# JonasGeiping/breaching

Measured on AMD Instinct MI355X. Metric: attack iters/sec, ResNet-18 ImageNet invertinggradients; PSNR vs ref, higher is better.
Workload: dtype f32

## Files before the change

breaching_amd/_lib.py:

```python

import ctypes
import os
from ctypes import POINTER, Structure, c_char_p, c_double, c_float, c_int, c_int32, c_int64, c_uint32, c_void_p

from . import build as _build

BH_ABI_VERSION = 8
BH_GM_CHUNK = 4096
BH_GM_MAX_PTRS = 448
BH_GM_PARTIAL_STRIDE = 4
BH_GM_MAX_ROWS = 2048
BH_GM_DEFAULT_ROWS = 512
BH_GM_STAT_WORDS = 12
BH_PRIOR_MAX_GRID = 1024
BH_BN_MAX_LAYERS = 448
BH_MT_MAX_PTRS = 112
BH_BN_TILE = 4096
BH_PRIOR_PARTIAL_STRIDE = 2
BH_STATE_WORDS = 16
BH_SCHED_STRIDE = 4
GM_CACHE_AUTO, GM_CACHE_KEEP, GM_CACHE_STREAM, GM_CACHE_STREAM_ALL = 0, 1, 2, 3

GM_KINDS = {
    "cosine-similarity": 0,
    "masked-cosine-similarity": 1,
    "fast-cosine-similarity": 2,
    "angular": 3,
    "euclidean": 4,
    "l1": 5,
    "tag-euclidean": 6,
    "pearlmutter-loss": 7,
}
GM_STAT_PATCH_D, GM_STAT_PATCH_R, GM_STAT_FD_STEP, GM_STAT_FD_SCALE = 8, 9, 10, 11
STATE_IT, STATE_DEAD, STATE_FIRST_BAD, STATE_IMPROVED, STATE_MIN, STATE_TOTAL, STATE_GNORM = range(7)
SIGN_NONE, SIGN_HARD, SIGN_SOFT = 0, 1, 2


class GmChunk(Structure):
    _fields_ = [("flat_off", c_int64), ("tensor_off", c_int64), ("tensor", c_int32), ("len", c_int32)]


class BnLayer(Structure):
    _fields_ = [("flat_off", c_int64), ("sums_off", c_int64), ("chan_off", c_int32), ("B", c_int32), ("C", c_int32),
                ("HW", c_int32), ("S", c_int32), ("narrow", c_int32), ("weight", c_float), ("div_unit_mul", c_uint32),
                ("div_unit_shr", c_uint32), ("div_c_mul", c_uint32), ("div_c_shr", c_uint32), ("fwd_items", c_int32)]


class BnItem(Structure):
    _fields_ = [("layer", c_int32), ("a", c_int32), ("b", c_int32), ("c", c_int32)]


class PsnrParams(Structure):
    _fields_ = [("mean", c_float * 4), ("std", c_float * 4), ("factor", c_float), ("clip", c_int32)]


class StepParams(Structure):
    _fields_ = [
        ("n", c_int64),
        ("plane", c_int64),
        ("channels", c_int32),
# ... 13 lines not shown

BH_STEP_MAX_SLOTS = 4


class StepSlot(Structure):
    _fields_ = [("params", StepParams), ("x", c_void_p), ("g", c_void_p), ("g_reg", c_void_p), ("noise", c_void_p), ("m", c_void_p),
                ("v", c_void_p), ("best", c_void_p)]


_PROTOTYPES = {
    "bh_abi_version": (c_int32, []),
    "bh_build_arch": (c_char_p, []),
    "bh_gm_num_groups": (c_int32, [c_int32]),
    "bh_gm_table_size": (c_int, [c_int32, POINTER(c_int64), POINTER(c_int64), POINTER(c_int64)]),
    "bh_gm_build_table": (c_int, [c_int32, POINTER(c_int64), POINTER(GmChunk), c_int64, POINTER(c_int64)]),
    "bh_gm_group_bounds": (c_int, [c_int32, POINTER(GmChunk), c_int64, POINTER(c_int32)]),
    "bh_gm_fwd": (
        c_int,
        [c_int32, c_int32, POINTER(c_void_p), c_void_p, c_void_p, c_int64, POINTER(c_int32), c_void_p, c_float, c_void_p,
         c_int32, c_int32, c_void_p, c_void_p, c_void_p],
    ),
    "bh_gm_fwd_rows": (c_int32, [c_int32, POINTER(c_int32), c_int32]),
    "bh_gm_finalize": (
        c_int,
        [c_int32, c_void_p, c_int64, c_float, c_float, c_float, c_float, c_void_p, c_void_p, c_void_p, c_void_p, c_void_p],
    ),
    "bh_wall_clock_khz": (c_int32, []),
    "bh_gm_bwd": (
        c_int,
        [c_int32, c_int32, POINTER(c_void_p), c_void_p, c_void_p, c_int64, POINTER(c_int32), c_void_p, c_void_p, c_void_p, c_void_p, c_int32,
         c_void_p, c_void_p, c_void_p],
    ),
    "bh_gm_pack": (c_int, [c_int32, POINTER(c_void_p), c_void_p, c_int64, POINTER(c_int32), c_void_p, c_void_p]),
    "bh_prior_tv_norm": (
        c_int,
        [c_void_p, c_int32, c_int32, c_int32, c_float, c_float, c_float, c_float, c_int32, c_float, c_float, c_void_p, c_void_p, c_void_p],
    ),
    "bh_bn_plan_size": (
        c_int,
        [c_int32, POINTER(c_int32), POINTER(c_int32), POINTER(c_int32), POINTER(c_int64), POINTER(c_int64), POINTER(c_int64),
         POINTER(c_int64), POINTER(c_int64)],
    ),
    "bh_bn_plan_build": (
        c_int,
        [c_int32, POINTER(c_int32), POINTER(c_int32), POINTER(c_int32), POINTER(c_float), POINTER(BnLayer), POINTER(BnItem),
         c_int64, POINTER(BnItem), c_int64],
    ),
    "bh_bn_bwd_accumulate": (c_int, [c_void_p, c_void_p, c_int32, c_void_p, c_void_p, c_int64, c_void_p, c_void_p, c_void_p, c_void_p]),
    "bh_bn_eval_fwd": (c_int, [c_void_p] * 8 + [c_int32, c_int32, c_int32, c_int32, c_void_p]),
    "bh_bn_eval_slabs": (c_int32, [c_int32, c_int32, c_int32]),
    "bh_bn_eval_bwd": (c_int, [c_void_p] * 14 + [c_int32, c_int32, c_int32, c_void_p]),
    "bh_bn_eval_bwd_bwd": (c_int, [c_void_p] * 14 + [c_int32, c_int32, c_int32, c_void_p]),
    "bh_bn_eval_bwd_bwd2": (c_int, [c_void_p] * 15 + [c_int32, c_int32, c_int32, c_void_p]),
    "bh_ln_fwd": (c_int, [c_void_p] * 6 + [c_int32, c_int32, ctypes.c_float, c_void_p]),
    "bh_ln_bwd": (c_int, [c_void_p] * 8 + [c_int32, c_int32, c_void_p]),
    "bh_ln_bwd_bwd": (c_int, [c_void_p] * 12 + [c_int32, c_int32, c_void_p]),
    "bh_bn_sums": (c_int, [c_int32, POINTER(c_void_p), POINTER(c_int32), c_void_p, c_void_p, c_int64, c_void_p, c_int32, c_int32, c_void_p]),
    "bh_bn_finalize": (c_int, [c_int32, c_void_p, c_void_p, c_void_p, c_void_p, c_void_p, c_void_p, c_void_p, c_void_p, c_int32, c_void_p]),
    "bh_bn_bwd": (
        c_int,
        [c_int32, POINTER(c_void_p), POINTER(c_int32), c_void_p, c_void_p, c_int64, c_void_p, c_void_p, c_void_p, c_void_p],
    ),
    "bh_mt_num_groups": (c_int32, [c_int32]),
    "bh_mt_group_bounds": (c_int, [c_int32, POINTER(GmChunk), c_int64, POINTER(c_int32)]),
    "bh_mt_axpy": (
        c_int,
        [c_int32, POINTER(c_void_p), POINTER(c_void_p), POINTER(c_void_p), c_float, c_void_p, c_int64, POINTER(c_int32), c_void_p,
         c_void_p],
    ),
    "bh_mt_scale": (c_int, [c_int32, POINTER(c_void_p), c_float, c_void_p, c_int64, POINTER(c_int32), c_void_p, c_void_p]),
    "bh_mt_patch": (
        c_int,
        [c_int32, POINTER(c_void_p), POINTER(c_void_p), c_void_p, c_void_p, c_float, c_void_p, c_int64, POINTER(c_int32), c_void_p,
         c_void_p],
    ),
    "bh_prior_orthogonality": (c_int, [c_void_p, c_int32, c_int64, c_void_p, c_void_p, c_void_p]),
    "bh_metric_psnr": (
        c_int,
        [c_void_p, c_void_p, c_int32, c_int64, c_int64, c_int32, POINTER(PsnrParams), c_void_p, c_void_p, c_void_p],
    ),
    "bh_event_create": (c_int, [POINTER(c_void_p)]),
    "bh_event_destroy": (c_int, [c_void_p]),
    "bh_event_record": (c_int, [c_void_p, c_void_p]),
    "bh_event_elapsed_ms": (c_int, [c_void_p, c_void_p, POINTER(c_float)]),
    "bh_state_reset": (c_int, [c_void_p, c_void_p]),
    "bh_loss_commit": (c_int, [c_void_p, c_void_p, c_int32, c_void_p, c_void_p, c_int32, c_void_p, c_void_p, c_void_p]),
    "bh_grad_norm": (c_int, [c_void_p, c_void_p, c_void_p, c_void_p, c_int64, c_void_p, c_float, c_void_p, c_void_p]),
    "bh_trial_key": (c_int64, [c_float, c_int32]),
    "bh_trial_key_unpack": (c_int, [c_int64, POINTER(c_float), POINTER(c_int32)]),
    "bh_step_list_norm_rows": (c_int32, [c_int32, POINTER(StepSlot)]),
    "bh_grad_norm_list": (c_int, [c_void_p, c_int32, POINTER(StepSlot), c_void_p, c_void_p, c_void_p]),
    "bh_candidate_step_list": (c_int, [c_void_p, c_void_p, c_int32, POINTER(StepSlot), c_void_p, c_void_p]),
    "bh_candidate_step": (
        c_int,
        [c_void_p, c_void_p, POINTER(StepParams), c_void_p, c_void_p, c_void_p, c_void_p, c_void_p, c_void_p, c_void_p, c_void_p],
    ),
}

EXPORTED_SYMBOLS = tuple(_PROTOTYPES)

_LIB = None


class BreachHipError(RuntimeError):
    """A C-ABI call returned a non-zero status."""

# ... 47 lines not shown
```

breaching_amd/attacker.py:

```python

import copy
import logging
import time
from collections import defaultdict

import numpy as np
import torch

from . import _lib, schedules, streams as trial_streams, trials, workers
from .config import cfg_get as _cfg_get
from .gm import objective_lookup
from .priors import HipNormRegularization, HipTotalVariation, launch_tv_norm, regularizer_lookup
from .victim_layers import (FusedEpilogueError, _ConvFunction, _ConvGradFunction, _EvalAffineBatchNorm2d, _EvalBNFunction,
                            _EvalBNGradFunction, _HipConv2d, _HipLayerNorm, owned_conv_grad_enabled, use_owned_conv_gradient,
                            _launch_eval_bn, _LayerNormFunction, _LayerNormGradFunction, _PendingBatchNorm, _under_functorch,
                            fast_eval_bn_enabled, fast_eval_bn_mode, fast_layer_norm_enabled, fuse_bn_relu_enabled, fuse_bn_relu_policy,
                            use_affine_eval_batchnorm, use_hip_layernorm)

log = logging.getLogger(__name__)

embedding_layer_names = ["encoder.weight", "word_embeddings.weight", "transformer.wte"]

_DEFAULT_SETUP = dict(dtype=torch.float, device=torch.device("cpu"))


class HipOptimizationAttacker:

    def __init__(self, model, loss_fn, cfg_attack, setup=_DEFAULT_SETUP):
        self.cfg = cfg_attack
        self.memory_format = torch.channels_last if cfg_attack.impl.mixed_precision else torch.contiguous_format
        self.setup = dict(device=torch.device(setup["device"]), dtype=getattr(torch, cfg_attack.impl.dtype))
        if self.setup["device"].type != "cuda":
            raise RuntimeError(
                f"HipOptimizationAttacker needs a ROCm device (setup['device']={self.setup['device']}); the HIP hot "
                "path has no CPU fallback. Use the reference attacker for CPU runs."
            )
        if self.setup["dtype"] != torch.float32 or cfg_attack.impl.mixed_precision:
            raise NotImplementedError("The HIP hot path computes in fp32 (impl.dtype=float, mixed_precision=False).")
        _lib.load()
        self.model_template = copy.deepcopy(model)
        self.loss_fn = copy.deepcopy(loss_fn)

        objective_cls = objective_lookup.get(self.cfg.objective.type)
        if objective_cls is None:
            raise ValueError(f"Unknown objective type {self.cfg.objective.type} given.")
        self.objective = objective_cls(**self.cfg.objective)

        self.regularizers = []
        regs = _cfg_get(self.cfg, "regularization")
        if regs is not None and hasattr(regs, "keys"):
            for key in regs.keys():
                if regs[key].scale > 0:
                    self.regularizers.append(regularizer_lookup[key](self.setup, **regs[key]))
        for reg in self.regularizers:
            if hasattr(reg, "tuning"):
                reg.tuning = {name: int(_cfg_get(self.cfg.impl, f"bn_{name}") or 0) for name in ("grid_cap", "load_depth", "finalize_block")}

        augs = _cfg_get(self.cfg, "augmentations")
        if augs is not None and hasattr(augs, "keys") and len(list(augs.keys())) > 0:
            self.augmentations = self._build_augmentations(augs, setup)
        else:
            self.augmentations = torch.nn.Sequential()

    @staticmethod
    def _build_augmentations(augs, setup):
        try:
            from breaching.attacks.auxiliaries.augmentations import augmentation_lookup
# ... 48 lines not shown
                pool.ship("starts", dict(labels=labels, inits={t: tuple(inits[t]) for t in range(num_trials) if t % pool.world != 0}),
                          self.setup["device"])
                pool.submit([dict(dryrun=dryrun)] * (pool.world - 1))
            timing["prepare_s"] = time.perf_counter() - t_call

            local_scores, local_solutions = {}, {}
            group_runs = None
            mine = list(shard.local_trials())
            width = trials_in_flight(self.cfg) if (self._fused_loop_supported() and not noisy) else 1
            try:
                for start in range(0, len(mine), max(width, 1)):
                    group = mine[start : start + max(width, 1)]
                    t_group = time.perf_counter()
                    if len(group) == 1:
                        solutions = {group[0]: self._run_trial(rec_models, shared_data, labels, stats, group[0], initial_data,
                                                               dryrun, init_state=inits.get(group[0]))}
                    else:
                        solutions, group_runs = self._run_trial_group(rec_models, shared_data, labels, stats, group, initial_data, dryrun,
                                                                      {t: inits[t] for t in group}, reuse=group_runs)
                    t_score = time.perf_counter()
                    timing["trials_s"] += t_score - t_group
                    for trial, solution in solutions.items():
                        local_solutions[trial] = solution
                        local_scores[trial] = self._score_trial(self._solution_data(solution),
                                                                self._score_labels(solution, labels), rec_models, shared_data)
                    timing["score_s"] += time.perf_counter() - t_score
            except KeyboardInterrupt:
                print("Trial procedure manually interruped.")
            if pool is not None:
                t_wait = time.perf_counter()
                pool.expect("trials_done")
                pool.timing["trials_wait_s"] = round(time.perf_counter() - t_wait, 4)
                pool.broadcast(("go",))
            before_select = getattr(self, "_before_select", None)
            if before_select is not None:
                before_select()
            stats["execution_trials"] = dict(self._trial_execution)
            t_select = time.perf_counter()
            optimal = self._select_optimal_reconstruction(local_solutions, local_scores, stats, shard)
            timing["select_s"] = time.perf_counter() - t_select
            if pool is not None:
                pool.timing["select_s"] = round(timing["select_s"], 4)
                pool.finish()
        except BaseException:
            if pool is not None:
                pool.abort()
                if pool.closed:
                    self._pool = None
            raise
        timing["total_s"] = time.perf_counter() - t_call
        stats["execution"] = dict(trials=stats.pop("execution_trials"), pool=pool.describe() if pool is not None else None,
                                  fused_epilogue_fallback=getattr(self, "fused_epilogue_fallback", None),
                                  owned_conv_grad=owned_conv_grad_enabled(self.cfg),
                                  pool_fallback=getattr(self, "_pool_fallback", None), world=shard.world,
                                  trial_streams=trial_streams.calibration_report(self.setup["device"]),
                                  timing={k: round(v, 4) for k, v in timing.items()})
        reconstructed_data = self._package(optimal, labels)
        if server_payload[0]["metadata"].modality == "text":
            raw = reconstructed_data["data"]
            reconstructed_data = self._postprocess_text_data(reconstructed_data)
            self._attach_raw_embeddings(reconstructed_data, raw)
        if "ClassAttack" in server_secrets:
            true_num_data = server_secrets["ClassAttack"]["true_num_data"]
            full = torch.zeros([true_num_data, *self.data_shape], **self.setup)
            full[server_secrets["ClassAttack"]["target_indx"]] = optimal if torch.is_tensor(optimal) else optimal[0]
            reconstructed_data["data"] = full
            reconstructed_data["labels"] = server_secrets["ClassAttack"]["all_labels"]
        return reconstructed_data, stats

    def _trial_worker_pool(self, num_trials):
        import torch.distributed as dist

        if getattr(self, "_is_trial_worker", False) or num_trials < 2:
            return None
        pool = getattr(self, "_pool", None)
        if pool is not None and not pool.closed:
            return pool
        self._pool_fallback = None
        devices = workers.requested_devices(self.cfg, self.setup["device"])[:num_trials]
        if len(devices) < 2:
            return None
        foreign = workers.active_pool()
        if foreign is not None and not foreign.busy:
            log.info("Closing another attacker's idle trial worker pool.")
            foreign.close()
        if dist.is_available() and dist.is_initialized():
            return None
        template = copy.deepcopy(self.model_template).to("cpu")
        loss_fn = copy.deepcopy(self.loss_fn).to("cpu") if isinstance(self.loss_fn, torch.nn.Module) else self.loss_fn
        try:
            self._pool = workers.TrialWorkerPool(devices, workers.attacker_runner_factory,
                                                 (type(self).__name__, template, loss_fn, self.cfg))
        except Exception as exc:
            if _cfg_get(self.cfg.impl, "trial_pool", "auto") == "required":
                raise
            self._pool_fallback = f"could not start the trial workers on devices {devices}: {exc!r}"
            log.warning(f"{self._pool_fallback}; running every trial on {self.setup['device']}.")
            self._pool = None
        return self._pool

    def close(self):
        pool = getattr(self, "_pool", None)
        if pool is not None:
            pool.close()
            self._pool = None

# ... 35 lines not shown

        metadata = server_payload[0]["metadata"]
        self.data_shape = metadata.shape
        if hasattr(metadata, "mean"):
            self.dm = torch.as_tensor(metadata.mean, **self.setup)[None, :, None, None]
            self.ds = torch.as_tensor(metadata.std, **self.setup)[None, :, None, None]
        else:
            self.dm, self.ds = torch.tensor(0, **self.setup), torch.tensor(1, **self.setup)

        rec_models = self._construct_models_from_payload_and_buffers(server_payload, shared_data)
        shared_data = self._cast_shared_data(shared_data)
        if metadata.modality == "text":
            rec_models, shared_data = self._prepare_for_text_data(shared_data, rec_models)
        self._rec_models = rec_models
        if shared_data[0]["metadata"]["labels"] is None:
            labels = self._recover_label_information(shared_data, server_payload, rec_models)
        else:
            labels = shared_data[0]["metadata"]["labels"].clone().to(self.setup["device"])
        if self.cfg.normalize_gradients:
            shared_data = self._normalize_gradients(shared_data)
        return rec_models, labels, stats

    def _construct_models_from_payload_and_buffers(self, server_payload, shared_data):
        models = []
        for idx, payload in enumerate(server_payload):
            new_model = copy.deepcopy(self.model_template)
            new_model.to(**self.setup, memory_format=self.memory_format)
            if shared_data[idx]["buffers"] is not None:
                buffers = shared_data[idx]["buffers"]
                new_model.eval()
            elif payload["buffers"] is not None:
                buffers = payload["buffers"]
                new_model.eval()
            else:
                new_model.train()
                for module in new_model.modules():
                    if hasattr(module, "track_running_stats"):
                        module.reset_parameters()
                        module.track_running_stats = False
                buffers = []
            with torch.no_grad():
                for param, server_state in zip(new_model.parameters(), payload["parameters"]):
                    param.copy_(server_state.to(**self.setup))
                for buffer, server_state in zip(new_model.buffers(), buffers):
                    buffer.copy_(server_state.to(**self.setup))
            if self.cfg.impl.JIT is not None:
                raise NotImplementedError("impl.JIT (torch.jit script/trace of the victim model) is not supported.")
            bn_mode = fast_eval_bn_mode(self.cfg)
            if bn_mode is not None:
                use_affine_eval_batchnorm(new_model, bn_mode, fuse_epilogue=fuse_bn_relu_enabled(self.cfg))
            if fast_layer_norm_enabled(self.cfg):
                use_hip_layernorm(new_model)
            if owned_conv_grad_enabled(self.cfg):
                use_owned_conv_gradient(new_model)
            models.append(new_model)
        return models

    def _cast_shared_data(self, shared_data):
        for data in shared_data:
            data["gradients"] = [g.to(**self.setup) for g in data["gradients"]]
            if data["buffers"] is not None:
                data["buffers"] = [b.to(device=self.setup["device"], dtype=self.setup["dtype"]) for b in data["buffers"]]
        return shared_data

    def _normalize_gradients(self, shared_data, fudge_factor=1e-6):
        for data in shared_data:
            grad_norm = torch.stack([g.pow(2).sum() for g in data["gradients"]]).sum().sqrt()
            torch._foreach_div_(data["gradients"], max(grad_norm, fudge_factor))
        return shared_data

    def _prepare_for_text_data(self, shared_data, rec_models):
        if self.cfg.text_strategy == "run-embedding":
            self.embeddings = []
            for model, data in zip(rec_models, shared_data):
                names = [n for n, _ in model.named_parameters()]
                name_to_idx = dict(zip(names, range(len(data["gradients"]))))
                position = None
                for marker in embedding_layer_names:
                    for key in name_to_idx:
                        if marker in key:
                            position = name_to_idx[key]
                if position is None:
                    raise ValueError("Could not locate the token embedding among the model parameters.")
                weight = list(model.parameters())[position]
                self.embeddings.append(dict(weight=weight, grads=data["gradients"].pop(position)))

                def _disable(module, weight=weight):
                    for child_name, child in module.named_children():
                        if isinstance(child, torch.nn.Embedding):
                            if child.weight is weight:
                                setattr(module, child_name, torch.nn.Identity())
                        else:
                            _disable(child)

                _disable(model)
            _, token_embedding_dim = self.embeddings[0]["weight"].shape
            self.data_shape = [*self.data_shape, token_embedding_dim]
        elif self.cfg.text_strategy == "no-preprocessing":
            pass
        else:
            raise ValueError(f"Invalid text strategy {self.cfg.text_strategy} given.")
        return rec_models, shared_data

    def _postprocess_text_data(self, reconstructed_user_data, models=None):
        def _closest_token(recovered, table):
            recovered = recovered - recovered.mean(dim=-1, keepdim=True)
            table = table - table.mean(dim=-1, keepdim=True)
# ... 801 lines not shown
```

breaching_amd/build.py:

```python

import hashlib
import os
import shutil
import subprocess
import sys

PKG_DIR = os.path.dirname(os.path.abspath(__file__))
REPO_ROOT = os.path.dirname(PKG_DIR)
CSRC = os.path.join(PKG_DIR, "csrc")
INCLUDE = os.path.join(REPO_ROOT, "include")
LIB_DIR = os.path.join(PKG_DIR, "lib")
LIB_PATH = os.path.join(LIB_DIR, "libbreach_hip.so")
STAMP_PATH = os.path.join(LIB_DIR, "libbreach_hip.stamp")

SOURCES = ["gm_kernels.hip", "prior_kernels.hip", "step_kernels.hip", "mt_kernels.hip", "affine_kernels.hip", "layernorm_kernels.hip"]
HEADERS = [os.path.join(CSRC, "bh_common.h"), os.path.join(INCLUDE, "breach_hip.h")]
ARCH = "gfx950"
FLAGS = ["-O3", "-std=c++17", "-fPIC", "-shared", f"--offload-arch={ARCH}", "-fno-gpu-rdc", "-Wall", "-Wno-unused-function"]


def _hipcc():
    for cand in (os.environ.get("HIPCC"), shutil.which("hipcc"), "/opt/rocm/bin/hipcc"):
        if cand and os.path.exists(cand):
            return cand
    raise RuntimeError("hipcc not found; libbreach_hip.so cannot be built (set HIPCC=/path/to/hipcc)")


def source_digest():
    h = hashlib.sha256()
    for path in [os.path.join(CSRC, s) for s in SOURCES] + HEADERS:
        with open(path, "rb") as f:
            h.update(f.read())
    h.update(" ".join(FLAGS).encode())
    return h.hexdigest()


def is_current():
    if not (os.path.exists(LIB_PATH) and os.path.exists(STAMP_PATH)):
        return False
    with open(STAMP_PATH) as f:
        return f.read().strip() == source_digest()


def build_library(force=False, verbose=False):
    if not force and is_current():
        return LIB_PATH
    os.makedirs(LIB_DIR, exist_ok=True)
    cmd = [_hipcc(), *FLAGS, f"-I{INCLUDE}", f"-I{CSRC}", *[os.path.join(CSRC, s) for s in SOURCES], "-o", LIB_PATH]
    if verbose:
        print(" ".join(cmd), flush=True)
    proc = subprocess.run(cmd, capture_output=True, text=True)
    if proc.returncode != 0:
        raise RuntimeError(f"hipcc failed ({proc.returncode}):\n{proc.stdout}\n{proc.stderr}")
    if verbose and proc.stderr.strip():
        print(proc.stderr, file=sys.stderr)
    with open(STAMP_PATH, "w") as f:
        f.write(source_digest())
    return LIB_PATH


if __name__ == "__main__":
    path = build_library(force="--force" in sys.argv, verbose=True)
    print(path)
```

breaching_amd/victim_layers.py:

```python

import torch

from . import _lib
from .config import cfg_get as _cfg_get

def _vector_ready(t, hw):
    if not t.is_contiguous():
        t = t.contiguous()
    if hw % 4 == 0 and t.data_ptr() % 16:
        t = t.clone()
    return t


def _under_functorch(x):
    try:
        from torch._C._functorch import is_functorch_wrapped_tensor, peek_interpreter_stack

        return bool(is_functorch_wrapped_tensor(x)) or peek_interpreter_stack() is not None
    except Exception:
        return False


class _EvalBNFunction(torch.autograd.Function):

# ... 74 lines not shown
        lib = _lib.load()
        gy, x, weight, inv_std, mean_inv, *rest = ctx.saved_tensors
        mask = rest[0] if ctx.masked else None
        none = (None,) * 9
        ggx2 = _take_conv_term(ctx)
        if ggx is None:
            ggx, ggx2 = ggx2, None
        if ggx is None and ggw is None and ggb is None and ggr is None:
            return none
        if ctx.extra_terms:
            raise NotImplementedError("No derivative of the BatchNorm backward with the DeepInversion term / another gradient folded in.")
        B, C = x.shape[0], x.shape[1]
        hw = x[0, 0].numel()
        ggx = None if ggx is None else _vector_ready(ggx.to(torch.float32), hw)
        ggx2 = None if ggx2 is None else _vector_ready(ggx2.to(torch.float32), hw)
        ggr = None if ggr is None else _vector_ready(ggr.to(torch.float32), hw)
        ggw = None if ggw is None else ggw.to(torch.float32).contiguous()
        ggb = None if ggb is None else ggb.to(torch.float32).contiguous()
        d_gy = torch.empty_like(x) if ctx.needs_input_grad[0] else None
        d_x = torch.empty_like(x) if (ctx.needs_input_grad[1] and ggw is not None) else None
        d_w = torch.empty(C, dtype=torch.float32, device=x.device) if (weight is not None and ctx.needs_input_grad[2] and ggx is not None) else None
        if d_gy is None and d_x is None and d_w is None:
            return none
        slabs = lib.bh_bn_eval_slabs(B, C, hw)
        ws = torch.empty(C * slabs, dtype=torch.float64, device=x.device) if slabs > 1 else None
        with torch.cuda.device(x.device):
            _lib.check(lib.bh_bn_eval_bwd_bwd2(_lib.ptr(ggx), _lib.ptr(ggx2), _lib.ptr(ggw), _lib.ptr(ggb), _lib.ptr(gy), _lib.ptr(x),
                                               _lib.ptr(weight), _lib.ptr(inv_std), _lib.ptr(mean_inv), _lib.ptr(d_gy), _lib.ptr(d_x),
                                               _lib.ptr(d_w), _lib.ptr(ws), _lib.ptr(mask), _lib.ptr(ggr), B, C, hw,
                                               _lib.current_stream_handle(x.device)), "bh_bn_eval_bwd_bwd2")
        return d_gy, d_x, d_w, None, None, None, None, None, None


def _take_conv_term(node):
    entry = getattr(node, "_conv_term", None)
    if entry is None:
        return None
    node._conv_term = None
    return entry[1] if entry[0] == torch._C._current_graph_task_id() else None


def _engine_wants(edge):
    node = edge[0] if edge is not None else None
    if node is None:
        return False
    try:
        return bool(torch._C._will_engine_execute_node(node))
    except RuntimeError:
        return True


_aten = torch.ops.aten


class _ConvFunction(torch.autograd.Function):

    @staticmethod
    def forward(ctx, x, w, b, stride, padding, dilation, groups):
        ctx.geometry = (list(stride), list(padding), list(dilation), int(groups))
        ctx.bias_sizes = None if b is None else [w.shape[0]]
        ctx.save_for_backward(x, w)
        return _aten.convolution(x, w, b, ctx.geometry[0], ctx.geometry[1], ctx.geometry[2], False, [0] * len(ctx.geometry[0]), groups)

    @staticmethod
    def backward(ctx, gy):
        x, w = ctx.saved_tensors
        none = (None,) * 7
        mask = tuple(bool(ctx.needs_input_grad[i]) and _engine_wants(ctx.next_functions[i]) for i in range(3))
        if not any(mask):
            return none
        producer = gy.grad_fn if gy.output_nr == 0 and getattr(gy.grad_fn, "_forward_cls", None) is _EvalBNGradFunction else None
        gx, gw, gb = _ConvGradFunction.apply(gy, x, w, ctx.geometry, mask, ctx.bias_sizes, producer)
        return (gx, gw, gb) + none[3:]


class _ConvGradFunction(torch.autograd.Function):

    @staticmethod
    def forward(ctx, gy, x, w, geometry, mask, bias_sizes, producer):
        stride, padding, dilation, groups = geometry
        ctx.geometry, ctx.producer = geometry, producer
        ctx.save_for_backward(gy, x, w)
        ctx.set_materialize_grads(False)
        return _aten.convolution_backward(gy, x, w, bias_sizes, stride, padding, dilation, False, [0] * len(stride), groups, list(mask))

    @staticmethod
    @torch.autograd.function.once_differentiable
    def backward(ctx, ggx, ggw, ggb):
        gy, x, w = ctx.saved_tensors
        stride, padding, dilation, groups = ctx.geometry
        zeros = [0] * len(stride)
        want = [bool(ctx.needs_input_grad[i]) and _engine_wants(ctx.next_functions[i]) for i in range(3)]
        d_gy = d_x = d_w = None
        if want[0]:
            t1 = None if ggx is None else _aten.convolution(ggx, w, None, stride, padding, dilation, False, zeros, groups)
            t2 = None if ggw is None else _aten.convolution(x, ggw, None, stride, padding, dilation, False, zeros, groups)
            if t1 is not None and t2 is not None:
                d_gy = t1 if ggb is None and _leave_on_producer(ctx, t2) else t1 + t2
            else:
                d_gy = t1 if t2 is None else t2
            if ggb is not None:
                bias = ggb.reshape(1, -1, *([1] * (gy.dim() - 2)))
                d_gy = bias.expand_as(gy) if d_gy is None else d_gy + bias
        if want[1] and ggw is not None:
            d_x = _aten.convolution_backward(gy, x, ggw, None, stride, padding, dilation, False, zeros, groups, [True, False, False])[0]
        if want[2] and ggx is not None:
            d_w = _aten.convolution_backward(gy, ggx, w, None, stride, padding, dilation, False, zeros, groups, [False, True, False])[1]
        return d_gy, d_x, d_w, None, None, None, None


def _leave_on_producer(ctx, term):
    producer = ctx.producer
    if producer is None or ctx.next_functions[0] != (producer, 0):
        return False
    try:
        if not torch._C._will_engine_execute_node(producer):
            return False
    except RuntimeError:
        return False
    task = torch._C._current_graph_task_id()
    entry = getattr(producer, "_conv_term", None)
    if entry is not None and entry[0] == task:
        term = entry[1] + term
    producer._conv_term = (task, term)
    return True


class _HipConv2d(torch.nn.Conv2d):

    def forward(self, x):
        if isinstance(x, _PendingBatchNorm):
            x = x.value()
        if (self.padding_mode != "zeros" or isinstance(self.padding, str) or x.dim() != 4 or not x.is_floating_point()
                or x.dtype != self.weight.dtype or torch.is_autocast_enabled(x.device.type) or _under_functorch(x)):
            return super().forward(x)
        return _ConvFunction.apply(x, self.weight, self.bias, self.stride, self.padding, self.dilation, self.groups)


def use_owned_conv_gradient(model):
    for module in model.modules():
        if type(module) is torch.nn.Conv2d:
            module.__class__ = _HipConv2d
    return model


def owned_conv_grad_enabled(cfg):
    import os

    env = os.environ.get("BREACH_HIP_CONV_GRAD")
    if env is not None:
        return env.strip().lower() not in ("0", "false", "off", "no")
    flag = _cfg_get(cfg.impl, "owned_conv_grad", True)
    return True if flag is None else bool(flag)


def _launch_eval_bn(module, x, sink, tap, residual, relu):
    inv_std, mean_inv = module._frozen_statistics()
    out = _EvalBNFunction.apply(x, module.weight, module.bias, inv_std, mean_inv, sink, tap, residual, relu)
    if tap is not None:
        tap.token = out[2]
    return out[0]


_RELU_OUT_OF_PLACE = (torch.relu, torch.nn.functional.relu, torch.Tensor.relu)
_RELU_IN_PLACE = (torch.relu_, torch.Tensor.relu_, torch.nn.functional.relu_)
_ADD_OUT_OF_PLACE = (torch.add, torch.Tensor.add, torch.Tensor.__add__, torch.Tensor.__radd__)
_ADD_IN_PLACE = (torch.Tensor.add_, torch.Tensor.__iadd__)


class FusedEpilogueError(RuntimeError):
    """The deferred BatchNorm launch (`_PendingBatchNorm`) met a consumer it cannot serve.  With cfg.impl.fuse_bn_relu = "auto" (the
    default) the attacker catches it on the model copy it happened on, switches the epilogue fusion off there and repeats the
    evaluation; "required" lets it through."""


class _PendingBatchNorm(torch.Tensor):

    @staticmethod
    def __new__(cls, module, x, sink, tap):
        self = torch.Tensor._make_wrapper_subclass(cls, x.shape, dtype=x.dtype, device=x.device, requires_grad=False)
        self._module, self._x, self._sink, self._tap = module, x, sink, tap
        self._residual, self._value = None, None
        self._graph_expected = torch.is_grad_enabled() and x.requires_grad
        if tap is not None:
            tap.pending = self
        return self

    def launch(self, relu=False):
        if self._graph_expected and not torch.is_grad_enabled():
            raise FusedEpilogueError("An eval-mode BatchNorm output was handed to a custom autograd.Function (or consumed inside a "
                                     "no_grad block) before any ordinary operation used it; the deferred BatchNorm launch cannot "
                                     "carry an autograd edge there.  cfg.impl.fuse_bn_relu='auto' (the default) falls back to "
                                     "un-fused launches on this model; False (or BREACH_HIP_FUSE_BN_RELU=0) never defers.")
        return _launch_eval_bn(self._module, self._x, self._sink, self._tap, self._residual, relu)

# ... 268 lines not shown
```

include/breach_hip.h:

```cpp
#ifndef BREACH_HIP_H
#define BREACH_HIP_H

#include <stdint.h>

#ifdef __cplusplus
extern "C" {
#endif

#define BH_ABI_VERSION 8
#define BH_EINVAL (-1)


#ifndef BH_GM_CHUNK
#define BH_GM_CHUNK 4096
#endif
#define BH_GM_MAX_PTRS 448
#define BH_GM_PARTIAL_STRIDE 4
#define BH_GM_MAX_ROWS 2048
#define BH_GM_DEFAULT_ROWS 512

typedef struct bh_gm_chunk {
  int64_t flat_off;
  int64_t tensor_off;
  int32_t tensor;
  int32_t len;
} bh_gm_chunk;

enum bh_gm_kind {
  BH_GM_COSINE = 0,
  BH_GM_COSINE_MASKED = 1,
  BH_GM_COSINE_FAST = 2,
  BH_GM_ANGULAR = 3,
  BH_GM_L2 = 4,
  BH_GM_L1 = 5,
  BH_GM_TAG = 6,
  BH_GM_PEARL_L2 = 7
};

enum bh_gm_stat {
  BH_GM_STAT_LOSS = 0,
  BH_GM_STAT_C1 = 1,
  BH_GM_STAT_C2 = 2,
  BH_GM_STAT_S0 = 3,
  BH_GM_STAT_S1 = 4,
  BH_GM_STAT_S2 = 5,
  BH_GM_STAT_SPAN_TICKS = 6,
  BH_GM_STAT_PATCH_D = 8,
  BH_GM_STAT_PATCH_R = 9,
  BH_GM_STAT_FD_STEP = 10,
  BH_GM_STAT_FD_SCALE = 11,
  BH_GM_STAT_WORDS = 12
};

int bh_gm_table_size(int32_t n_tensors, const int64_t* numel, int64_t* n_chunks, int64_t* flat_elems);

int bh_gm_build_table(int32_t n_tensors, const int64_t* numel, bh_gm_chunk* chunks, int64_t n_chunks,
                      int64_t* tensor_flat_off);

int bh_gm_fwd(int32_t kind, int32_t n_tensors, const void* const* rec_ptrs, const float* data_flat,
              const bh_gm_chunk* chunks_dev, int64_t n_chunks, const int32_t* group_chunk_begin,
              const float* weights_dev, float tag_scale, double* partials_dev, int32_t rows_cap, int32_t cache_policy,
              void* stream, void* ev_start, void* ev_stop);
// ... 45 lines not shown
  uint32_t div_unit_mul, div_unit_shr;
  uint32_t div_c_mul, div_c_shr;
  int32_t fwd_items;
} bh_bn_layer;

typedef struct bh_bn_item {
  int32_t layer, a, b, c;
} bh_bn_item;

int bh_bn_plan_size(int32_t n_layers, const int32_t* B, const int32_t* C, const int32_t* HW, int64_t* n_fwd_items,
                    int64_t* n_bwd_items, int64_t* flat_elems, int64_t* n_sum_pairs, int64_t* n_channels);
int bh_bn_plan_build(int32_t n_layers, const int32_t* B, const int32_t* C, const int32_t* HW, const float* weights,
                     bh_bn_layer* layers, bh_bn_item* fwd_items, int64_t n_fwd_items, bh_bn_item* bwd_items,
                     int64_t n_bwd_items);

int bh_bn_sums(int32_t n_layers, const void* const* x_ptrs, const int32_t* hw_host, const bh_bn_layer* layers_dev,
               const bh_bn_item* fwd_items_dev, int64_t n_fwd_items, double* sums_dev, int32_t grid_cap, int32_t load_depth,
               void* stream);

#define BH_BN_DEFAULT_FINALIZE_BLOCK 1024

int bh_bn_finalize(int32_t n_layers, const bh_bn_layer* layers_dev, const double* sums_dev, const float* running_mean,
                   const float* running_var, float* coef_dev, double* layer_values_dev, float* total_dev,
                   void* counter_dev, int32_t block_threads, void* stream);

int bh_bn_bwd(int32_t n_layers, const void* const* x_ptrs, const int32_t* hw_host, const bh_bn_layer* layers_dev,
              const bh_bn_item* bwd_items_dev, int64_t n_bwd_items, const float* coef_dev, const float* gout_dev,
              float* grad_flat, void* stream);

int bh_bn_bwd_accumulate(const float* x, const float* gin, int32_t hw, const bh_bn_layer* layers_dev,
                         const bh_bn_item* layer_bwd_items_dev, int64_t n_items, const float* coef_dev, const float* gout_dev,
                         float* out, void* stream);

int bh_bn_eval_fwd(const float* x, const float* weight, const float* bias, const float* inv_std, const float* mean_inv, float* y,
                   double* stats, const float* residual, int32_t relu, int32_t B, int32_t C, int32_t HW, void* stream);
int32_t bh_bn_eval_slabs(int32_t B, int32_t C, int32_t HW);
int bh_bn_eval_bwd(const float* gy, const float* x, const float* weight, const float* inv_std, const float* mean_inv, float* gx,
                   float* gw, float* gb, double* workspace, const float* tap_coef, const float* tap_gout, const float* y_mask,
                   float* g_residual, const float* gx_add, int32_t B, int32_t C, int32_t HW, void* stream);
int bh_bn_eval_bwd_bwd(const float* ggx, const float* ggw, const float* ggb, const float* gy, const float* x, const float* weight,
                       const float* inv_std, const float* mean_inv, float* d_gy, float* d_x, float* d_w, double* workspace,
                       const float* y_mask, const float* gg_residual, int32_t B, int32_t C, int32_t HW, void* stream);
int bh_bn_eval_bwd_bwd2(const float* ggx, const float* ggx2, const float* ggw, const float* ggb, const float* gy, const float* x,
                        const float* weight, const float* inv_std, const float* mean_inv, float* d_gy, float* d_x, float* d_w,
                        double* workspace, const float* y_mask, const float* gg_residual, int32_t B, int32_t C, int32_t HW, void* stream);

int bh_ln_fwd(const float* x, const float* gamma, const float* beta, float* y, float* mean, float* rstd, int32_t R, int32_t D,
              float eps, void* stream);
int bh_ln_bwd(const float* gy, const float* x, const float* gamma, const float* mean, const float* rstd, float* gx, float* ggamma,
              float* gbeta, int32_t R, int32_t D, void* stream);
int bh_ln_bwd_bwd(const float* u, const float* s, const float* t, const float* gy, const float* x, const float* gamma,
                  const float* mean, const float* rstd, float* d_gy, float* d_x, float* d_gamma, float* row_scalars, int32_t R,
                  int32_t D, void* stream);


#define BH_MT_MAX_PTRS 112
int32_t bh_mt_num_groups(int32_t n_tensors);
int bh_mt_group_bounds(int32_t n_tensors, const bh_gm_chunk* chunks_host, int64_t n_chunks, int32_t* group_chunk_begin);

int bh_mt_axpy(int32_t n_tensors, const void* const* a_ptrs, const void* const* b_ptrs, const void* const* c_ptrs,
               float alpha, const bh_gm_chunk* chunks_dev, int64_t n_chunks, const int32_t* group_chunk_begin,
               float* out_flat, void* stream);
int bh_mt_scale(int32_t n_tensors, const void* const* a_ptrs, float alpha, const bh_gm_chunk* chunks_dev, int64_t n_chunks,
                const int32_t* group_chunk_begin, float* out_flat, void* stream);
int bh_mt_patch(int32_t n_tensors, const void* const* theta_ptrs, const void* const* grad_ptrs, const float* data_flat,
                const float* coef_dev, float mult, const bh_gm_chunk* chunks_dev, int64_t n_chunks,
                const int32_t* group_chunk_begin, float* out_flat, void* stream);

int bh_prior_orthogonality(const float* x, int32_t B, int64_t D, float* grad_out, double* partials_dev, void* stream);

typedef struct bh_psnr_params {
  float mean[4];
  float std[4];
  float factor;
  int32_t clip;
} bh_psnr_params;
int bh_metric_psnr(const float* rec, const float* ref, int32_t B, int64_t per_example, int64_t plane, int32_t channels,
                   const bh_psnr_params* params, double* mse_dev, float* out_dev, void* stream);


enum bh_state_word {
  BH_STATE_IT = 0,
  BH_STATE_DEAD = 1,
  BH_STATE_FIRST_BAD = 2,
  BH_STATE_IMPROVED = 3,
  BH_STATE_MIN = 4,
  BH_STATE_TOTAL = 5,
  BH_STATE_GNORM = 6,
  BH_STATE_WORDS = 16
};

int bh_state_reset(void* state_dev, void* stream);

int bh_loss_commit(void* state_dev, float* history_dev, int32_t history_len, const float* gm_loss,
                   const double* reg_partials, int32_t n_reg, const float* extra0, const float* extra1, void* stream);

int bh_grad_norm(void* state_dev, const float* g, const float* g_reg, const float* noise, int64_t n,
                 const double* sched_dev, float langevin, double* ws_dev, void* stream);

#define BH_SCHED_STRIDE 4

enum bh_sign_mode { BH_SIGN_NONE = 0, BH_SIGN_HARD = 1, BH_SIGN_SOFT = 2 };

typedef struct bh_step_params {
  int64_t n;
  int64_t plane;
// ... 49 lines not shown
```

Before: 113.9.

## Add native HIP direct convolution kernels for selected conv forward and backward-data

Adds hand-written HIP convolution kernels for forward and backward-data, tiled over output pixels and channels with the reduction dimension split across waves and summed in shared memory. They are routed in for bias-free 1x1 convs (forward only) and stride-1 3x3 convs with up to 64 reduction channels, including the double-backward path. Other shapes fall back to aten/MIOpen. The aim is to beat the library for the small-channel ResNet-18 convs, at the cost of plain FP32 FMA code with no matrix-core use and more custom kernels to maintain.

After: 113.6. Within noise of the previous version (-0.3%).

```diff
diff --git a/breaching_amd/_lib.py b/breaching_amd/_lib.py
--- a/breaching_amd/_lib.py
+++ b/breaching_amd/_lib.py
@@ -5,7 +5,7 @@
 
 from . import build as _build
 
-BH_ABI_VERSION = 8
+BH_ABI_VERSION = 9
 BH_GM_CHUNK = 4096
 BH_GM_MAX_PTRS = 448
 BH_GM_PARTIAL_STRIDE = 4
@@ -125,6 +125,9 @@
     "bh_bn_eval_bwd": (c_int, [c_void_p] * 14 + [c_int32, c_int32, c_int32, c_void_p]),
     "bh_bn_eval_bwd_bwd": (c_int, [c_void_p] * 14 + [c_int32, c_int32, c_int32, c_void_p]),
     "bh_bn_eval_bwd_bwd2": (c_int, [c_void_p] * 15 + [c_int32, c_int32, c_int32, c_void_p]),
+    "bh_conv2d_fwd": (c_int, [c_void_p] * 3 + [c_int32] * 14 + [c_void_p]),
+    "bh_conv2d_bwd_data": (c_int, [c_void_p] * 3 + [c_int32] * 14 + [c_void_p]),
+    "bh_conv2d_selected": (c_int32, [c_int32] * 12),
     "bh_ln_fwd": (c_int, [c_void_p] * 6 + [c_int32, c_int32, ctypes.c_float, c_void_p]),
     "bh_ln_bwd": (c_int, [c_void_p] * 8 + [c_int32, c_int32, c_void_p]),
     "bh_ln_bwd_bwd": (c_int, [c_void_p] * 12 + [c_int32, c_int32, c_void_p]),
diff --git a/breaching_amd/attacker.py b/breaching_amd/attacker.py
--- a/breaching_amd/attacker.py
+++ b/breaching_amd/attacker.py
@@ -12,7 +12,7 @@
 from .gm import objective_lookup
 from .priors import HipNormRegularization, HipTotalVariation, launch_tv_norm, regularizer_lookup
 from .victim_layers import (FusedEpilogueError, _ConvFunction, _ConvGradFunction, _EvalAffineBatchNorm2d, _EvalBNFunction,
-                            _EvalBNGradFunction, _HipConv2d, _HipLayerNorm, owned_conv_grad_enabled, use_owned_conv_gradient,
+                            _EvalBNGradFunction, _HipConv2d, _HipLayerNorm, native_conv_enabled, owned_conv_grad_enabled, use_owned_conv_gradient,
                             _launch_eval_bn, _LayerNormFunction, _LayerNormGradFunction, _PendingBatchNorm, _under_functorch,
                             fast_eval_bn_enabled, fast_eval_bn_mode, fast_layer_norm_enabled, fuse_bn_relu_enabled, fuse_bn_relu_policy,
                             use_affine_eval_batchnorm, use_hip_layernorm)
@@ -167,6 +167,7 @@
         stats["execution"] = dict(trials=stats.pop("execution_trials"), pool=pool.describe() if pool is not None else None,
                                   fused_epilogue_fallback=getattr(self, "fused_epilogue_fallback", None),
                                   owned_conv_grad=owned_conv_grad_enabled(self.cfg),
+                                  native_conv=owned_conv_grad_enabled(self.cfg) and native_conv_enabled(self.cfg),
                                   pool_fallback=getattr(self, "_pool_fallback", None), world=shard.world,
                                   trial_streams=trial_streams.calibration_report(self.setup["device"]),
                                   timing={k: round(v, 4) for k, v in timing.items()})
@@ -308,7 +309,7 @@
             if fast_layer_norm_enabled(self.cfg):
                 use_hip_layernorm(new_model)
             if owned_conv_grad_enabled(self.cfg):
-                use_owned_conv_gradient(new_model)
+                use_owned_conv_gradient(new_model, native_conv=native_conv_enabled(self.cfg))
             models.append(new_model)
         return models
 
diff --git a/breaching_amd/build.py b/breaching_amd/build.py
--- a/breaching_amd/build.py
+++ b/breaching_amd/build.py
@@ -13,7 +13,8 @@
 LIB_PATH = os.path.join(LIB_DIR, "libbreach_hip.so")
 STAMP_PATH = os.path.join(LIB_DIR, "libbreach_hip.stamp")
 
-SOURCES = ["gm_kernels.hip", "prior_kernels.hip", "step_kernels.hip", "mt_kernels.hip", "affine_kernels.hip", "layernorm_kernels.hip"]
+SOURCES = ["gm_kernels.hip", "prior_kernels.hip", "step_kernels.hip", "mt_kernels.hip", "affine_kernels.hip", "layernorm_kernels.hip",
+           "conv_kernels.hip"]
 HEADERS = [os.path.join(CSRC, "bh_common.h"), os.path.join(INCLUDE, "breach_hip.h")]
 ARCH = "gfx950"
 FLAGS = ["-O3", "-std=c++17", "-fPIC", "-shared", f"--offload-arch={ARCH}", "-fno-gpu-rdc", "-Wall", "-Wno-unused-function"]
diff --git a/breaching_amd/csrc/conv_kernels.hip b/breaching_amd/csrc/conv_kernels.hip
--- /dev/null
+++ b/breaching_amd/csrc/conv_kernels.hip
@@ -0,0 +1,258 @@
+
+#include "bh_common.h"
+
+namespace {
+
+using bh::kBlock;
+
+constexpr int kTileP = bh::kWave;
+constexpr int kSplits = bh::kWavesPerBlock;
+
+struct ConvGeom {
+  int32_t N;
+  int32_t Cr, M;
+  int32_t Hs, Ws;
+  int32_t Hd, Wd;
+  int32_t R, S, sh, sw, ph, pw;
+};
+
+template <int DIR>
+__device__ __forceinline__ bool tap_position(const ConvGeom& g, int hd, int wd, int r, int s, int& off) {
+  int hs, ws;
+  bool ok;
+  if (DIR == 0) {
+    hs = hd * g.sh - g.ph + r;
+    ws = wd * g.sw - g.pw + s;
+    ok = hs >= 0 && ws >= 0;
+  } else {
+    const int nh = hd + g.ph - r, nw = wd + g.pw - s;
+    ok = nh >= 0 && nw >= 0;
+    hs = nh / g.sh;
+    ws = nw / g.sw;
+    ok = ok && hs * g.sh == nh && ws * g.sw == nw;
+  }
+  ok = ok && hs < g.Hs && ws < g.Ws;
+  off = ok ? hs * g.Ws + ws : 0;
+  return ok;
+}
+
+template <int DIR, int R, int S, int TM, int U>
+__global__ __launch_bounds__(kBlock) void conv_tile_kernel(const float* __restrict__ src, const float* __restrict__ w,
+                                                           float* __restrict__ dst, const ConvGeom g) {
+  constexpr int RS = R * S;
+  __shared__ float lds[kSplits * TM * kTileP];
+  const int lane = threadIdx.x & (kTileP - 1);
+  const int wave = __builtin_amdgcn_readfirstlane(threadIdx.x >> 6);
+  const int m0 = blockIdx.y * TM;
+  const int Ps = g.Hs * g.Ws, Pd = g.Hd * g.Wd;
+  const int n = blockIdx.x * kTileP + lane;
+  const bool live = n < g.N;
+  const int b = live ? n / Pd : 0;
+  const int p = live ? n - b * Pd : 0;
+  const int hd = p / g.Wd, wd = p - hd * g.Wd;
+
+  unsigned off[RS];
+  bool ok[RS];
+#pragma unroll
+  for (int r = 0; r < R; ++r) {
+#pragma unroll
+    for (int s = 0; s < S; ++s) {
+      int o;
+      ok[r * S + s] = tap_position<DIR>(g, hd, wd, r, s, o) && live;
+      off[r * S + s] = 4u * (unsigned)(b * g.Cr * Ps + o);
+    }
+  }
+  auto fetch_b = [&](int c0, float (&bv)[U * RS]) {
+#pragma unroll
+    for (int u = 0; u < U; ++u) {
+      const int c = c0 + u < g.Cr ? c0 + u : g.Cr - 1;
+      const unsigned plane = 4u * (unsigned)(c * Ps);
+#pragma unroll
+      for (int t = 0; t < RS; ++t) {
+        const float v = *reinterpret_cast<const float*>(reinterpret_cast<const char*>(src) + (off[t] + plane));
+        bv[u * RS + t] = ok[t] ? v : 0.f;
+      }
+    }
+  };
+
+  auto fetch_w = [&](int c0, float (&wv)[TM * U * RS]) {
+#pragma unroll
+    for (int u = 0; u < U; ++u) {
+      const bool have = c0 + u < g.Cr;
+      const int c = have ? c0 + u : 0;
+#pragma unroll
+      for (int m = 0; m < TM; ++m) {
+        const int mm = m0 + m < g.M ? m0 + m : g.M - 1;
+        const float* wt = w + (DIR == 0 ? mm * g.Cr + c : c * g.M + mm) * RS;
+#pragma unroll
+        for (int t = 0; t < RS; ++t) wv[(m * U + u) * RS + t] = have ? wt[t] : 0.f;
+      }
+    }
+  };
+
+  float acc[TM];
+#pragma unroll
+  for (int m = 0; m < TM; ++m) acc[m] = 0.f;
+  const int steps = (g.Cr + U - 1) / U;
+  constexpr bool kAhead = TM * U * RS * 2 <= 36;
+  float bcur[U * RS], bnext[U * RS];
+  float wcur[TM * U * RS], wnext[TM * U * RS];
+  if (wave < steps) {
+    fetch_b(wave * U, bcur);
+    if (kAhead) fetch_w(wave * U, wcur);
+  }
+  for (int i = wave; i < steps; i += kSplits) {
+    const bool more = i + kSplits < steps;
+    if (more) fetch_b((i + kSplits) * U, bnext);
+    if (kAhead) {
+      if (more) fetch_w((i + kSplits) * U, wnext);
+#pragma unroll
+      for (int u = 0; u < U; ++u) {
+#pragma unroll
+        for (int m = 0; m < TM; ++m) {
+#pragma unroll
+          for (int t = 0; t < RS; ++t) acc[m] = fmaf(wcur[(m * U + u) * RS + t], bcur[u * RS + t], acc[m]);
+        }
+      }
+    } else {
+#pragma unroll
+      for (int u = 0; u < U; ++u) {
+        const bool have = i * U + u < g.Cr;
+        const int c = have ? i * U + u : 0;
+#pragma unroll
+        for (int m = 0; m < TM; ++m) {
+          const int mm = m0 + m < g.M ? m0 + m : g.M - 1;
+          const float* wt = w + (DIR == 0 ? mm * g.Cr + c : c * g.M + mm) * RS;
+#pragma unroll
+          for (int t = 0; t < RS; ++t) acc[m] = fmaf(have ? wt[t] : 0.f, bcur[u * RS + t], acc[m]);
+        }
+      }
+    }
+#pragma unroll
+    for (int k = 0; k < U * RS; ++k) bcur[k] = bnext[k];
+    if (kAhead) {
+#pragma unroll
+      for (int k = 0; k < TM * U * RS; ++k) wcur[k] = wnext[k];
+    }
+  }
+#pragma unroll
+  for (int m = 0; m < TM; ++m) lds[(wave * TM + m) * kTileP + lane] = acc[m];
+  __syncthreads();
+  for (int m = wave; m < TM; m += kSplits) {
+    float s = lds[m * kTileP + lane];
+#pragma unroll
+    for (int k = 1; k < kSplits; ++k) s += lds[(k * TM + m) * kTileP + lane];
+    if (live && m0 + m < g.M) dst[(b * g.M + m0 + m) * Pd + p] = s;
+  }
+}
+
+template <int DIR>
+__global__ __launch_bounds__(kBlock) void conv_direct_kernel(const float* __restrict__ src, const float* __restrict__ w,
+                                                             float* __restrict__ dst, const ConvGeom g, const int32_t total) {
+  const int idx = blockIdx.x * kBlock + threadIdx.x;
+  if (idx >= total) return;
+  const int Ps = g.Hs * g.Ws, Pd = g.Hd * g.Wd;
+  const int p = idx % Pd;
+  const int bm = idx / Pd;
+  const int m = bm % g.M, b = bm / g.M;
+  const int hd = p / g.Wd, wd = p - hd * g.Wd;
+  const int RS = g.R * g.S;
+  const float* srcb = src + (int64_t)b * g.Cr * Ps;
+  float acc = 0.f;
+  for (int c = 0; c < g.Cr; ++c) {
+    const float* wc = DIR == 0 ? w + ((int64_t)m * g.Cr + c) * RS : w + ((int64_t)c * g.M + m) * RS;
+    const float* plane = srcb + (int64_t)c * Ps;
+    for (int r = 0; r < g.R; ++r) {
+      for (int s = 0; s < g.S; ++s) {
+        int off;
+        if (tap_position<DIR>(g, hd, wd, r, s, off)) acc = fmaf(wc[r * g.S + s], plane[off], acc);
+      }
+    }
+  }
+  dst[idx] = acc;
+}
+
+constexpr int64_t kIndexLimit = (int64_t)1 << 30;
+constexpr int64_t kFillWorkgroups = 512;
+constexpr int32_t kSelectMaxChannels = 64;
+
+bool conv_problem(const void* a, const void* w, const void* out, int32_t B, int32_t C, int32_t H, int32_t W, int32_t K, int32_t R,
+                  int32_t S, int32_t sh, int32_t sw, int32_t ph, int32_t pw, int32_t dh, int32_t dw, int32_t groups, int32_t& OH,
+                  int32_t& OW) {
+  if (!a || !w || !out) return false;
+  if (groups != 1 || dh != 1 || dw != 1) return false;
+  if (B < 1 || C < 1 || H < 1 || W < 1 || K < 1 || R < 1 || S < 1 || sh < 1 || sw < 1 || ph < 0 || pw < 0) return false;
+  const int64_t eh = (int64_t)H + 2 * (int64_t)ph - R, ew = (int64_t)W + 2 * (int64_t)pw - S;
+  if (eh < 0 || ew < 0) return false;
+  const int64_t oh = eh / sh + 1, ow = ew / sw + 1;
+  const int64_t limit = kIndexLimit - 4 * kBlock;
+  if ((int64_t)R * S >= limit || (int64_t)H * W >= limit || oh * ow >= limit) return false;
+  if ((int64_t)B * C * H * W >= limit || (int64_t)B * K * oh * ow >= limit || (int64_t)K * C * R * S >= limit) return false;
+  if ((int64_t)H + 2 * (int64_t)ph + R >= limit || (int64_t)W + 2 * (int64_t)pw + S >= limit) return false;
+  if (oh * sh + R >= limit || ow * sw + S >= limit) return false;
+  OH = (int32_t)oh, OW = (int32_t)ow;
+  return true;
+}
+
+template <int DIR>
+int conv_launch(const float* src, const float* w, float* dst, const ConvGeom& g, void* stream) {
+  hipStream_t st = bh::as_stream(stream);
+  const bool tile3 = g.R == 3 && g.S == 3, tile1 = g.R == 1 && g.S == 1;
+  const int64_t tiles_p = ((int64_t)g.N + kTileP - 1) / kTileP;
+  int tm = tile3 ? 8 : 4;
+  while (tm > 2 && tiles_p * (((int64_t)g.M + tm - 1) / tm) < kFillWorkgroups) tm >>= 1;
+  const int64_t tiles_m = ((int64_t)g.M + tm - 1) / tm;
+  if ((tile3 || tile1) && tiles_m <= 65535) {
+    const dim3 grid((unsigned)tiles_p, (unsigned)tiles_m), block(kBlock);
+#define BH_CONV_TILE(TM)                                                                                       \
+  if (tile3) hipLaunchKernelGGL((conv_tile_kernel<DIR, 3, 3, TM, 1>), grid, block, 0, st, src, w, dst, g); \
+  else hipLaunchKernelGGL((conv_tile_kernel<DIR, 1, 1, TM, 8>), grid, block, 0, st, src, w, dst, g)
+    if (tm == 8) { hipLaunchKernelGGL((conv_tile_kernel<DIR, 3, 3, 8, 1>), grid, block, 0, st, src, w, dst, g); }
+    else if (tm == 4) { BH_CONV_TILE(4); }
+    else { BH_CONV_TILE(2); }
+#undef BH_CONV_TILE
+  } else {
+    const int64_t total = (int64_t)g.N * g.M;
+    hipLaunchKernelGGL((conv_direct_kernel<DIR>), dim3((unsigned)((total + kBlock - 1) / kBlock)), dim3(kBlock), 0, st, src, w, dst, g,
+                       (int32_t)total);
+  }
+  return bh::launch_status();
+}
+
+}
+
+extern "C" {
+
+int bh_conv2d_fwd(const float* x, const float* w, float* y, int32_t B, int32_t C, int32_t H, int32_t W, int32_t K, int32_t R, int32_t S,
+                  int32_t stride_h, int32_t stride_w, int32_t pad_h, int32_t pad_w, int32_t dil_h, int32_t dil_w, int32_t groups,
+                  void* stream) {
+  int32_t OH, OW;
+  if (!conv_problem(x, w, y, B, C, H, W, K, R, S, stride_h, stride_w, pad_h, pad_w, dil_h, dil_w, groups, OH, OW)) return BH_EINVAL;
+  ConvGeom g;
+  g.N = B * OH * OW, g.Cr = C, g.M = K, g.Hs = H, g.Ws = W, g.Hd = OH, g.Wd = OW;
+  g.R = R, g.S = S, g.sh = stride_h, g.sw = stride_w, g.ph = pad_h, g.pw = pad_w;
+  return conv_launch<0>(x, w, y, g, stream);
+}
+
+int bh_conv2d_bwd_data(const float* gy, const float* w, float* dx, int32_t B, int32_t C, int32_t H, int32_t W, int32_t K, int32_t R,
+                       int32_t S, int32_t stride_h, int32_t stride_w, int32_t pad_h, int32_t pad_w, int32_t dil_h, int32_t dil_w,
+                       int32_t groups, void* stream) {
+  int32_t OH, OW;
+  if (!conv_problem(gy, w, dx, B, C, H, W, K, R, S, stride_h, stride_w, pad_h, pad_w, dil_h, dil_w, groups, OH, OW)) return BH_EINVAL;
+  ConvGeom g;
+  g.N = B * H * W, g.Cr = K, g.M = C, g.Hs = OH, g.Ws = OW, g.Hd = H, g.Wd = W;
+  g.R = R, g.S = S, g.sh = stride_h, g.sw = stride_w, g.ph = pad_h, g.pw = pad_w;
+  return conv_launch<1>(gy, w, dx, g, stream);
+}
+
+int32_t bh_conv2d_selected(int32_t backward_data, int32_t B, int32_t C, int32_t H, int32_t W, int32_t K, int32_t R, int32_t S,
+                           int32_t stride_h, int32_t stride_w, int32_t pad_h, int32_t pad_w) {
+  int32_t OH, OW;
+  const void* ok = &OH;
+  if (!conv_problem(ok, ok, ok, B, C, H, W, K, R, S, stride_h, stride_w, pad_h, pad_w, 1, 1, 1, OH, OW)) return 0;
+  if (R == 1 && S == 1) return backward_data ? 0 : 1;
+  const int32_t walked = backward_data ? K : C;
+  return R == 3 && S == 3 && stride_h == 1 && stride_w == 1 && walked <= kSelectMaxChannels ? 1 : 0;
+}
+
+}
diff --git a/breaching_amd/victim_layers.py b/breaching_amd/victim_layers.py
--- a/breaching_amd/victim_layers.py
+++ b/breaching_amd/victim_layers.py
@@ -150,20 +150,85 @@
 
 _aten = torch.ops.aten
 
+_NATIVE_CONV_FORCE = False
+
+
+def native_conv_enabled(cfg=None):
+    import os
+
+    env = os.environ.get("BREACH_HIP_NATIVE_CONV")
+    if env is not None:
+        return env.strip().lower() not in ("0", "false", "off", "no")
+    flag = _cfg_get(cfg.impl, "native_conv", True) if cfg is not None else True
+    return True if flag is None else bool(flag)
+
+
+def _native_conv_route(backward_data, x_shape, w, tensors, stride, padding, dilation, groups, native=None):
+    if not (native_conv_enabled() if native is None else native):
+        return None
+    if len(stride) != 2 or groups != 1 or tuple(dilation) != (1, 1) or w.dim() != 4:
+        return None
+    for t in tensors:
+        if not (t.is_cuda and t.dtype == torch.float32 and t.dim() == 4 and t.is_contiguous()) or _under_functorch(t):
+            return None
+    lib = _lib.load()
+    if not _NATIVE_CONV_FORCE and not lib.bh_conv2d_selected(int(backward_data), x_shape[0], x_shape[1], x_shape[2], x_shape[3], w.shape[0],
+                                                              w.shape[2], w.shape[3], stride[0], stride[1], padding[0], padding[1]):
+        return None
+    return lib
+
+
+def _native_conv_fwd(lib, x, w, stride, padding):
+    B, C, H, W = x.shape
+    K, _, R, S = w.shape
+    y = torch.empty((B, K, (H + 2 * padding[0] - R) // stride[0] + 1, (W + 2 * padding[1] - S) // stride[1] + 1), dtype=x.dtype, device=x.device)
+    with torch.cuda.device(x.device):
+        _lib.check(lib.bh_conv2d_fwd(_lib.ptr(x), _lib.ptr(w), _lib.ptr(y), B, C, H, W, K, R, S, stride[0], stride[1], padding[0], padding[1],
+                                     1, 1, 1, _lib.current_stream_handle(x.device)), "bh_conv2d_fwd")
+    return y
+
+
+def _native_conv_bwd_data(lib, gy, w, x_shape, stride, padding):
+    B, C, H, W = x_shape
+    K, _, R, S = w.shape
+    dx = torch.empty((B, C, H, W), dtype=gy.dtype, device=gy.device)
+    with torch.cuda.device(gy.device):
+        _lib.check(lib.bh_conv2d_bwd_data(_lib.ptr(gy), _lib.ptr(w), _lib.ptr(dx), B, C, H, W, K, R, S, stride[0], stride[1], padding[0],
+                                          padding[1], 1, 1, 1, _lib.current_stream_handle(gy.device)), "bh_conv2d_bwd_data")
+    return dx
+
+
+def _conv_fwd(x, w, stride, padding, dilation, groups, native=None):
+    x, w = x.detach(), w.detach()
+    lib = _native_conv_route(0, x.shape, w, (x, w), stride, padding, dilation, groups, native)
+    if lib is not None:
+        return _native_conv_fwd(lib, x, w, stride, padding)
+    return _aten.convolution(x, w, None, stride, padding, dilation, False, [0] * len(stride), groups)
+
+
+def _conv_bwd_data(gy, x, w, stride, padding, dilation, groups, native=None):
+    gy, w = gy.detach(), w.detach()
+    lib = _native_conv_route(1, x.shape, w, (gy, w), stride, padding, dilation, groups, native)
+    if lib is not None:
+        return _native_conv_bwd_data(lib, gy, w, x.shape, stride, padding)
+    return _aten.convolution_backward(gy, x, w, None, stride, padding, dilation, False, [0] * len(stride), groups, [True, False, False])[0]
+
 
 class _ConvFunction(torch.autograd.Function):
 
     @staticmethod
-    def forward(ctx, x, w, b, stride, padding, dilation, groups):
-        ctx.geometry = (list(stride), list(padding), list(dilation), int(groups))
+    def forward(ctx, x, w, b, stride, padding, dilation, groups, native=None):
+        ctx.geometry = (list(stride), list(padding), list(dilation), int(groups), native)
         ctx.bias_sizes = None if b is None else [w.shape[0]]
         ctx.save_for_backward(x, w)
+        if b is None:
+            return _conv_fwd(x, w, *ctx.geometry)
         return _aten.convolution(x, w, b, ctx.geometry[0], ctx.geometry[1], ctx.geometry[2], False, [0] * len(ctx.geometry[0]), groups)
 
     @staticmethod
     def backward(ctx, gy):
         x, w = ctx.saved_tensors
-        none = (None,) * 7
+        none = (None,) * 8
         mask = tuple(bool(ctx.needs_input_grad[i]) and _engine_wants(ctx.next_functions[i]) for i in range(3))
         if not any(mask):
             return none
@@ -176,23 +241,32 @@
 
     @staticmethod
     def forward(ctx, gy, x, w, geometry, mask, bias_sizes, producer):
-        stride, padding, dilation, groups = geometry
+        stride, padding, dilation, groups = geometry[:4]
+        native = geometry[4] if len(geometry) > 4 else None
         ctx.geometry, ctx.producer = geometry, producer
         ctx.save_for_backward(gy, x, w)
         ctx.set_materialize_grads(False)
+        if mask[0] and _native_conv_route(1, x.shape, w, (gy.detach(), w.detach()), stride, padding, dilation, groups, native) is not None:
+            gx = _conv_bwd_data(gy, x, w, stride, padding, dilation, groups, native)
+            gw = gb = None
+            if mask[1] or mask[2]:
+                _, gw, gb = _aten.convolution_backward(gy, x, w, bias_sizes, stride, padding, dilation, False, [0] * len(stride), groups,
+                                                       [False, bool(mask[1]), bool(mask[2])])
+            return gx, gw, gb
         return _aten.convolution_backward(gy, x, w, bias_sizes, stride, padding, dilation, False, [0] * len(stride), groups, list(mask))
 
     @staticmethod
     @torch.autograd.function.once_differentiable
     def backward(ctx, ggx, ggw, ggb):
         gy, x, w = ctx.saved_tensors
-        stride, padding, dilation, groups = ctx.geometry
+        stride, padding, dilation, groups = ctx.geometry[:4]
+        native = ctx.geometry[4] if len(ctx.geometry) > 4 else None
         zeros = [0] * len(stride)
         want = [bool(ctx.needs_input_grad[i]) and _engine_wants(ctx.next_functions[i]) for i in range(3)]
         d_gy = d_x = d_w = None
         if want[0]:
-            t1 = None if ggx is None else _aten.convolution(ggx, w, None, stride, padding, dilation, False, zeros, groups)
-            t2 = None if ggw is None else _aten.convolution(x, ggw, None, stride, padding, dilation, False, zeros, groups)
+            t1 = None if ggx is None else _conv_fwd(ggx, w, stride, padding, dilation, groups, native)
+            t2 = None if ggw is None else _conv_fwd(x, ggw, stride, padding, dilation, groups, native)
             if t1 is not None and t2 is not None:
                 d_gy = t1 if ggb is None and _leave_on_producer(ctx, t2) else t1 + t2
             else:
@@ -201,7 +275,7 @@
                 bias = ggb.reshape(1, -1, *([1] * (gy.dim() - 2)))
                 d_gy = bias.expand_as(gy) if d_gy is None else d_gy + bias
         if want[1] and ggw is not None:
-            d_x = _aten.convolution_backward(gy, x, ggw, None, stride, padding, dilation, False, zeros, groups, [True, False, False])[0]
+            d_x = _conv_bwd_data(gy, x, ggw, stride, padding, dilation, groups, native)
         if want[2] and ggx is not None:
             d_w = _aten.convolution_backward(gy, ggx, w, None, stride, padding, dilation, False, zeros, groups, [False, True, False])[1]
         return d_gy, d_x, d_w, None, None, None, None
@@ -232,13 +306,16 @@
         if (self.padding_mode != "zeros" or isinstance(self.padding, str) or x.dim() != 4 or not x.is_floating_point()
                 or x.dtype != self.weight.dtype or torch.is_autocast_enabled(x.device.type) or _under_functorch(x)):
             return super().forward(x)
-        return _ConvFunction.apply(x, self.weight, self.bias, self.stride, self.padding, self.dilation, self.groups)
-
-
-def use_owned_conv_gradient(model):
+        return _ConvFunction.apply(x, self.weight, self.bias, self.stride, self.padding, self.dilation, self.groups,
+                                   self.__dict__.get("native_conv"))
+
+
+def use_owned_conv_gradient(model, native_conv=None):
     for module in model.modules():
         if type(module) is torch.nn.Conv2d:
             module.__class__ = _HipConv2d
+        if type(module) is _HipConv2d:
+            module.native_conv = None if native_conv is None else bool(native_conv)
     return model
 
 
diff --git a/include/breach_hip.h b/include/breach_hip.h
--- a/include/breach_hip.h
+++ b/include/breach_hip.h
@@ -7,7 +7,7 @@
 extern "C" {
 #endif
 
-#define BH_ABI_VERSION 8
+#define BH_ABI_VERSION 9
 #define BH_EINVAL (-1)
 
 
@@ -159,6 +159,15 @@
 int bh_ln_bwd_bwd(const float* u, const float* s, const float* t, const float* gy, const float* x, const float* gamma,
                   const float* mean, const float* rstd, float* d_gy, float* d_x, float* d_gamma, float* row_scalars, int32_t R,
                   int32_t D, void* stream);
+
+int bh_conv2d_fwd(const float* x, const float* w, float* y, int32_t B, int32_t C, int32_t H, int32_t W, int32_t K, int32_t R, int32_t S,
+                  int32_t stride_h, int32_t stride_w, int32_t pad_h, int32_t pad_w, int32_t dil_h, int32_t dil_w, int32_t groups,
+                  void* stream);
+int bh_conv2d_bwd_data(const float* gy, const float* w, float* dx, int32_t B, int32_t C, int32_t H, int32_t W, int32_t K, int32_t R,
+                       int32_t S, int32_t stride_h, int32_t stride_w, int32_t pad_h, int32_t pad_w, int32_t dil_h, int32_t dil_w,
+                       int32_t groups, void* stream);
+int32_t bh_conv2d_selected(int32_t backward_data, int32_t B, int32_t C, int32_t H, int32_t W, int32_t K, int32_t R, int32_t S,
+                           int32_t stride_h, int32_t stride_w, int32_t pad_h, int32_t pad_w);
 
 
 #define BH_MT_MAX_PTRS 112
```
